# CaNS-World/CaLES

Measured on AMD Instinct MI355X. Metric: time-steps/sec, higher is better.
Workload: dtype f64; 1 GPU; turbulent channel 512x512x512, sgstype=dsmag, PP/PP/NN pressure BCs, bulk forcing in x (BASELINE.json configs[2]); 3 RK substeps/step; decomposition=single GPU

## Files before the change

### cales_amd/csrc/common.hpp

```cpp
#pragma once
#include <hip/hip_runtime.h>
#include <cstdint>
#include <cstdio>
#include <cstdlib>
#include <cstring>
#include <cmath>
#include <string>
#include <vector>
#include "../../include/cales.h"

typedef cales_real real;
#ifdef CALES_SINGLE
typedef float2 real2;
#define CALES_EPS 1.1920929e-07f
#define CALES_BIG 3.4028235e38f
#else
typedef double2 real2;
#define CALES_EPS 2.220446049250313e-16
#define CALES_BIG 1.7976931348623157e308
#endif
constexpr int RSZ = (int)sizeof(real);
constexpr int LINE_REALS = 128 / RSZ;
__host__ __device__ inline real2 make_real2(real x, real y) { real2 r; r.x = x; r.y = y; return r; }

struct Geom {
  int n1, n2, n3;
  int s1;
  long s12;
  int jlo;
  int ng2;

  __host__ __device__ inline size_t ix(int i, int j, int k) const { return (size_t)i + (size_t)s1 * (size_t)j + (size_t)s12 * (size_t)k; }
};

struct DBound { real *x = nullptr, *y = nullptr, *z = nullptr; };
struct RhsBz {
  const real *bc; char ctype, cf; real dlc, dlf, sgn, alpha;
  __host__ __device__ inline real at(int i, int j, int n1) const {
    const real bcv = bc[i + (size_t)(n1 + 2) * j];
    real r = 0.;
    if (cf == 'c') { if (ctype == 'D') r = -2. * bcv / dlc / dlf; else if (ctype == 'N') r = sgn * bcv / dlf; }
    else           { if (ctype == 'D') r = -bcv / dlc / dlf;      else if (ctype == 'N') r = sgn * bcv / dlc; }
    return r * alpha;
  }
};

struct Comm {
  cales_halo_cb halo = nullptr; cales_alltoall_cb a2a = nullptr; cales_allreduce_cb allred = nullptr; void *user = nullptr;
  real *A = nullptr, *B = nullptr; int64_t nbuf = 0;
  bool on = false;
  cales_halo_s_cb halo_s = nullptr; cales_alltoall_part_cb a2a_part = nullptr;
  bool halo_second_stream = false, a2a_second_stream = false, has_lo = false, has_hi = false;
};

struct Spec {
  int blocked, cw, n2l, n3;
  int nyq = 0;
  __host__ __device__ inline size_t at_slab(const Geom &g, int m, int jl, int k) const {
    if (!blocked) return (g.ix(0, jl, k) >> 1) + (size_t)m;
    const int peer = m / cw, mm = m - peer * cw;
    return (size_t)mm + (size_t)cw * ((size_t)(jl - 1) + (size_t)n2l * ((size_t)(k - 1) + (size_t)n3 * peer));
  }
  __host__ __device__ inline size_t at_mode(const Geom &g, int mm, int j, int k) const {
    if (!blocked) return (g.ix(0, j, k) >> 1) + (size_t)mm;
    const int peer = (j - 1) / n2l, jl = (j - 1) - peer * n2l;
    return (size_t)mm + (size_t)cw * ((size_t)jl + (size_t)n2l * ((size_t)(k - 1) + (size_t)n3 * peer));
  }
};

struct Flags {
  bool unfolded_correc = false, unfolded_mom = false, eager_projection = false, lazy_projection = false, helmholtz_z_per_column = false, unfused_imp_rhs = false, unfused_correc = false, unfused_forcing = false, unfused_fillps = false, unfused_mean = false, keep_last_rhs = false, wide_offsets = false, dsmag_reference_sequence = false, dsmag_xghosts = false, smag_reference_sequence = false, gaussel_march = false, fft_generic = false, fft_no_odd_radix = false, keep_null_mode = false, unfused_rk = false, overlap = false, xghosts_in_step = false, unmerged_bc = false, no_nyquist_packing = false, sgs_six_components = false;
  int kchunk = 0; long tile_min_blocks = 2048;
  std::string test_bad_launch;
  void read_env() {
    test_bad_launch = getenv("CALES_TEST_BAD_LAUNCH") ? getenv("CALES_TEST_BAD_LAUNCH") : "";
    unfolded_mom = getenv("CALES_UNFOLDED_MOM") != nullptr;
    lazy_projection = getenv("CALES_LAZY_PROJECTION") != nullptr;
    eager_projection = getenv("CALES_EAGER_PROJECTION") != nullptr;
    unfolded_correc = getenv("CALES_UNFOLDED_CORREC") != nullptr;
    helmholtz_z_per_column = getenv("CALES_HELMHOLTZ_Z_PER_COLUMN") != nullptr;
    unfused_imp_rhs = getenv("CALES_UNFUSED_IMP_RHS") != nullptr;
    unfused_correc = getenv("CALES_UNFUSED_CORREC") != nullptr;
    unfused_forcing = getenv("CALES_UNFUSED_FORCING") != nullptr;
    unfused_fillps = getenv("CALES_UNFUSED_FILLPS") != nullptr;
    unfused_mean = getenv("CALES_UNFUSED_MEAN") != nullptr;
    keep_last_rhs = getenv("CALES_KEEP_LAST_RHS") != nullptr;
    wide_offsets = getenv("CALES_WIDE_OFFSETS") != nullptr;
    dsmag_reference_sequence = getenv("CALES_DSMAG_REFERENCE_SEQUENCE") != nullptr;
    dsmag_xghosts = getenv("CALES_DSMAG_XGHOSTS") != nullptr;
    sgs_six_components = getenv("CALES_SGS_SIX_COMPONENTS") != nullptr;
    smag_reference_sequence = getenv("CALES_SMAG_REFERENCE_SEQUENCE") != nullptr;
    gaussel_march = getenv("CALES_GAUSSEL_MARCH") != nullptr;
    no_nyquist_packing = getenv("CALES_NO_NYQUIST_PACKING") != nullptr;
    fft_generic = getenv("CALES_FFT_GENERIC") != nullptr;
    fft_no_odd_radix = getenv("CALES_FFT_NO_ODD_RADIX") != nullptr;
    xghosts_in_step = getenv("CALES_XGHOSTS_IN_STEP") != nullptr;
    keep_null_mode = getenv("CALES_KEEP_NULL_MODE") != nullptr;
    unfused_rk = getenv("CALES_UNFUSED_RK") != nullptr;
    overlap = getenv("CALES_OVERLAP") != nullptr && atoi(getenv("CALES_OVERLAP")) != 0 && getenv("CALES_NO_OVERLAP") == nullptr;
    unmerged_bc = getenv("CALES_UNMERGED_BC") != nullptr;
    kchunk = getenv("CALES_KCHUNK") ? atoi(getenv("CALES_KCHUNK")) : 0;
    tile_min_blocks = getenv("CALES_TILE_MIN_BLOCKS") ? atol(getenv("CALES_TILE_MIN_BLOCKS")) : 2048;
  }
};

struct StepPlan {
  bool valid = false;
  bool in_visct_zero = false, in_sgs_first = false;
  bool xskip = false;
  bool fold_correc = false;
  bool fold_rows2 = false;
  bool fold_mom = false;
  bool lazy_last = false;
  bool defer_imp_rhs = false;
  bool any_wm = false, skip_first_wm = false;
  bool fuse_cu = false;
  bool defer_force = false;
  bool fuse_fill = false;
  bool visct_ghosts = false;
  bool keep_last_rhs = false;
  int mean_mask = 0, force_mask = 0;
};

struct BandMap { int gx, gy, gz, sub; };
struct TileGeom { dim3 block, grid; int kchunk = 0; BandMap bm{0, 0, 0, 0}; };

enum class SgsForm { none, smag_rows, smag_reference, dsmag_tiles, dsmag_reference };
enum class StrainKernel { corr_rows2, corr, corr5, yw32, yw64, pair, plain32, plain64, f2d32, f2d64 };
enum class LmfKernel { pair, pair5, yw_ucf32, yw_ucf64, yw32, yw64, ucf32, ucf64, plain32, plain64, f2d32, f2d64 };
enum class SmagKernel { yw32, yw64, plain32, plain64 };
enum class SgsAve { planes, volume, xlines };
struct SgsPath {
  SgsForm form = SgsForm::none;
  bool pair = false, lazy = false, ucf = false, small = false, yw = false;
  bool five = false;
  bool filter2d = false;
  SgsAve ave = SgsAve::planes;
  bool wraps_x = true;
  int zlo = 0, zhi = 0, wmlo = 0, wmhi = 0, wylo = 0, wyhi = 0, wmylo = 0, wmyhi = 0; real flo = 0., fhi = 0.;
  int perz = 0, perx = 0, skipz = 0, lmf_ty = 0;
  StrainKernel strain = StrainKernel::plain64; LmfKernel lmf = LmfKernel::plain64; SmagKernel smag = SmagKernel::plain64;
  TileGeom strain_geo, corr_geo, corr_rows2_geo, lmf_geo, smag_geo;
};
struct SgsFold { real dtrk; bool rows2; int fmask; };

struct MomPath {
  bool fused = true;
  int imp = 0;
  bool small = false;
  TileGeom geo;
  bool wm = false, wm_ghosts_in_step = false;
};
struct PendingProjection { real dtrk = 0.; int fmask = 0; bool p_done = false, xskip = false; };

struct BcRule { char t0, t1, cen; real dr0, dr1; const real *bc0, *bc1; };
// ... 329 lines not shown
```

### cales_amd/csrc/k_solver.hip

```cpp
#include "common.hpp"

struct __attribute__((aligned(2 * sizeof(real)))) cpx { real x, y; };
__device__ inline cpx cadd(cpx a, cpx b) { return {a.x + b.x, a.y + b.y}; }
__device__ inline cpx csub(cpx a, cpx b) { return {a.x - b.x, a.y - b.y}; }
__device__ inline cpx cmul(cpx a, cpx b) { return {a.x * b.x - a.y * b.y, a.x * b.y + a.y * b.x}; }
__device__ inline cpx cconj(cpx a) { return {a.x, -a.y}; }
template <int INV> __device__ inline cpx mul_mi(cpx a) { return INV ? cpx{-a.y, a.x} : cpx{a.y, -a.x}; }

template <int R, int INV>
__device__ inline void fft_stage(const cpx *__restrict__ in, cpx *__restrict__ out, int N, int Ns, int t, int T, const cpx *__restrict__ tw) {
  const int M = N / R, tstep = N / (Ns * R);
  for (int j = t; j < M; j += T) {
    const int k = j % Ns;
    cpx v[R];
#pragma unroll
    for (int r = 0; r < R; ++r) v[r] = in[j + r * M];
    if (Ns > 1) {
#pragma unroll
      for (int r = 1; r < R; ++r) { cpx w = tw[k * r * tstep]; if (INV) w.y = -w.y; v[r] = cmul(v[r], w); }
    }
    const int j0 = (j - k) * R + k;
    if (R == 2) {
      out[j0] = cadd(v[0], v[1]); out[j0 + Ns] = csub(v[0], v[1]);
    } else if (R == 4) {
// ... 197 lines not shown
#pragma unroll
    for (int b = 0; b < 4; ++b) { buf[lpad(j0[b])] = v[b][0]; buf[lpad(j0[b] + Ns)] = v[b][1]; }
    __syncthreads();
  }
}

__device__ inline int lmap(int i) { return i; }
template <int INV>
__device__ inline void fft_line8_dif(int N, cpx *buf, int t, const cpx *__restrict__ tw, cpx *v) {
  const int T = N >> 3;
  int R0 = N; while ((R0 & 7) == 0) R0 >>= 3;
  int Nsp;
  if (R0 == 1) {
    fft8_regs<INV>(v);
    if (T == 1) return;
#pragma unroll
    for (int r = 1; r < 8; ++r) v[r] = tw_mul<INV>(v[r], tw[t * r]);
    Nsp = T >> 3;
  } else if (R0 == 4) {
#pragma unroll
    for (int b = 0; b < 2; ++b) {
      const cpx a0 = cadd(v[b], v[b + 4]), a1 = csub(v[b], v[b + 4]), a2 = cadd(v[b + 2], v[b + 6]), a3 = mul_mi<INV>(csub(v[b + 2], v[b + 6]));
      const int j = t + b * T;
      v[b] = cadd(a0, a2); v[b + 2] = tw_mul<INV>(cadd(a1, a3), tw[j]); v[b + 4] = tw_mul<INV>(csub(a0, a2), tw[2 * j]); v[b + 6] = tw_mul<INV>(csub(a1, a3), tw[3 * j]);
    }
    Nsp = T >> 2;
  } else {
#pragma unroll
    for (int b = 0; b < 4; ++b) {
      const cpx x0 = v[b], x1 = v[b + 4];
      v[b] = cadd(x0, x1); v[b + 4] = tw_mul<INV>(csub(x0, x1), tw[t + b * T]);
    }
    Nsp = T >> 1;
  }
  while (true) {
#pragma unroll
    for (int e = 0; e < 8; ++e) buf[lmap(t + e * T)] = v[e];
    __syncthreads();
    const int k = t % Nsp, base = (t - k) * 8 + k, tstep = N / (Nsp * 8);
#pragma unroll
    for (int r = 0; r < 8; ++r) v[r] = buf[lmap(base + r * Nsp)];
    fft8_regs<INV>(v);
    if (Nsp == 1) break;
#pragma unroll
    for (int r = 1; r < 8; ++r) v[r] = tw_mul<INV>(v[r], tw[k * r * tstep]);
    __syncthreads();
    Nsp >>= 3;
  }
}

__device__ inline int dct_src(int e, int n) { return e < n / 2 ? 2 * e : 2 * (n - 1 - e) + 1; }
struct FillArgs { const real *u, *v, *w, *dzfi; real dti, dtidxi, dtidyi; int mean_mask; const real *gvr_f, *gvr_c; real *part; int pstride = 0, pofs = 0; int xwrap = 0; };
template <int INV, int KIND, int FILL = 0, int ODD = 0>
__global__ __launch_bounds__(256, (KIND == 1 && FILL == 1) ? 2 : 1) void k_fft_x8(Geom g, int nh, int iters, const cpx *__restrict__ twg, const cpx *__restrict__ twpg,
                                                 const cpx *__restrict__ twd, real *__restrict__ p, real scale, Spec S, real2 *__restrict__ spec,
                                                 FillArgs F = FillArgs{}, long rbeg = 0, long rend = -1) {
  extern __shared__ __align__(16) unsigned char smem[];
  constexpr int kind = KIND;
  const int T = nh >> 3, R = blockDim.x / T, row = threadIdx.x / T, t = threadIdx.x % T, ld = lpad(nh) + 2;
  cpx *tw = reinterpret_cast<cpx *>(smem), *twp = tw + nh;
  cpx *twl = twp + nh + 1;
  cpx *A = twl + (kind ? nh + 1 : 0) + (size_t)row * ld;
  for (int q = threadIdx.x; q < nh; q += blockDim.x) tw[q] = twg[q];
  for (int q = threadIdx.x; q <= nh; q += blockDim.x) twp[q] = twpg[q];
  if (kind) for (int q = threadIdx.x; q <= nh; q += blockDim.x) twl[q] = twd[q];
  const long nrows = rend < 0 ? (long)g.n2 * g.n3 : rend;
  const int NE = 8;
  cpx nxt[NE + 1];
  real macc[3] = {0., 0., 0.};
  auto rowptr = [&](long r, int &j, int &k) { j = (int)(r % g.n2) + 1; k = (int)(r / g.n2) + 1; };
  auto fetch = [&](long r) {
    if (r >= nrows) return;
    int j, k; rowptr(r, j, k);
    if (!INV && FILL) {
      const size_t c0 = g.ix(0, j, k);
      const real dz = F.dzfi[k];
#pragma unroll
      for (int e = 0; e < NE; ++e) {
        const size_t c = c0 + 1 + 2 * (t + e * T);
        const real2 uu = *reinterpret_cast<const real2 *>(F.u + c); const real um = (F.xwrap && t + e * T == 0) ? F.u[c0 + F.xwrap] : F.u[c - 1];
        const real2 vv = *reinterpret_cast<const real2 *>(F.v + c), vm = *reinterpret_cast<const real2 *>(F.v + c - g.s1);
        const real2 ww = *reinterpret_cast<const real2 *>(F.w + c), wm = *reinterpret_cast<const real2 *>(F.w + c - g.s12);
        nxt[e] = cpx{((ww.x - wm.x) * F.dti * dz + (vv.x - vm.x) * F.dtidyi + (uu.x - um) * F.dtidxi),
                     ((ww.y - wm.y) * F.dti * dz + (vv.y - vm.y) * F.dtidyi + (uu.y - uu.x) * F.dtidxi)};
        if (F.mean_mask & 1) macc[0] += (uu.x + uu.y) * F.gvr_f[k];
        if (F.mean_mask & 2) macc[1] += (vv.x + vv.y) * F.gvr_f[k];
        if (F.mean_mask & 4) macc[2] += (ww.x + ww.y) * F.gvr_c[k];
      }
    } else if (!INV) {
      const real *rowp = p + g.ix(0, j, k);
#pragma unroll
      for (int e = 0; e < NE; ++e) { const int q = t + e * T; nxt[e] = cpx{rowp[1 + 2 * q], rowp[2 + 2 * q]}; }
    } else if (!kind) {
#pragma unroll
      for (int e = 0; e < NE; ++e) { const real2 v = spec[S.at_slab(g, t + e * T, j, k)]; nxt[e] = cpx{v.x, v.y}; }
      if (t == 0) {
        if (S.nyq) { nxt[NE] = cpx{nxt[0].y, 0.}; nxt[0].y = 0.; }
        else { const real2 v = spec[S.at_slab(g, nh, j, k)]; nxt[NE] = cpx{v.x, v.y}; }
      }
    } else {
#pragma unroll
      for (int e = 0; e < NE; ++e) { const real2 v = spec[S.at_slab(g, t + e * T, j, k)]; nxt[e] = cpx{v.x, v.y}; }
    }
  };
  long r = rbeg + ((long)blockIdx.x * iters) * R + row;
  fetch(r);
  for (int it = 0; it < iters; ++it, r += R) {
    const bool live = r < nrows;
    int j = 1, k = 1; if (live) rowptr(r, j, k);
    if (kind && !INV) {
      real *Ad = reinterpret_cast<real *>(A);
#pragma unroll
      for (int e = 0; e < NE; ++e) {
        const int q = t + e * T, r = 2 * nh - 1 - q;
        Ad[2 * lpad(q >> 1) + (q & 1)] = nxt[e].x; Ad[2 * lpad(r >> 1) + (r & 1)] = nxt[e].y;
      }
    } else {
#pragma unroll
      for (int e = 0; e < NE; ++e) A[lpad(t + e * T)] = nxt[e];
    }
    if (INV && !kind && t == 0) A[lpad(nh)] = nxt[NE];
    __syncthreads();
    if (it + 1 < iters) fetch(r + R);
    if (INV && kind) {
      const real *Ad = reinterpret_cast<const real *>(A); const int n = 2 * nh;
      auto coef = [&](int kk) {
        const real yk = Ad[2 * lpad(kk >> 1) + (kk & 1)];
        const int r2 = n - kk; const real ym = kk == 0 ? 0. : Ad[2 * lpad(r2 >> 1) + (r2 & 1)];
        return cmul(cconj(twl[kk]), cpx{yk, -ym});
      };
      cpx xk[NE + 1];
#pragma unroll
      for (int e = 0; e < NE; ++e) xk[e] = coef(t + e * T);
      if (t == 0) xk[NE] = coef(nh);
      __syncthreads();
#pragma unroll
      for (int e = 0; e < NE; ++e) A[lpad(t + e * T)] = xk[e];
      if (t == 0) A[lpad(nh)] = xk[NE];
      __syncthreads();
    }
    real *rowp = p + g.ix(0, j, k);
    if (!INV) {
      fft_line8<0, ODD>(nh, A, t, tw);
      if (live) {
        for (int kk = t; kk <= nh / 2; kk += T) {
          const cpx zk = A[lpad(kk)], zm = cconj(A[lpad((nh - kk) % nh)]);
          const cpx E = {(real)(0.5 * (zk.x + zm.x)), (real)(0.5 * (zk.y + zm.y))};
          const cpx D = csub(zk, zm), O = {(real)(0.5 * D.y), (real)(-0.5 * D.x)};
          const cpx wO = cmul(twp[kk], O);
          const cpx xk = cadd(E, wO), xm = cconj(csub(E, wO));
          if (!kind) {
            if (S.nyq && kk == 0) spec[S.at_slab(g, 0, j, k)] = make_real2(xk.x, xm.x);
            else {
            spec[S.at_slab(g, kk, j, k)] = make_real2(xk.x, xk.y);
            spec[S.at_slab(g, nh - kk, j, k)] = make_real2(xm.x, xm.y);
            }
          } else {
            real *sd = reinterpret_cast<real *>(spec);
            const int n = 2 * nh, k2 = nh - kk;
            const cpx a = cmul(twl[kk], xk), b2 = cmul(twl[k2], xm);
            auto put = [&](int rr, real val) { if (rr < n) sd[2 * S.at_slab(g, rr >> 1, j, k) + (rr & 1)] = val; };
            put(kk, 2. * a.x); if (kk) put(n - kk, -2. * a.y);
            put(k2, 2. * b2.x); if (k2 && k2 != n - k2) put(n - k2, -2. * b2.y);
          }
        }
      }
    } else {
      for (int kk = t; kk <= nh / 2; kk += T) {
        const cpx xa = A[lpad(kk)], xb = A[lpad(nh - kk)];
        const cpx Sa = cadd(xa, cconj(xb)), Da = csub(xa, cconj(xb)), wa = cmul(cconj(twp[kk]), Da);
        const cpx Sb = cadd(xb, cconj(xa)), Db = csub(xb, cconj(xa)), wb = cmul(cconj(twp[nh - kk]), Db);
        const cpx za = cpx{Sa.x - wa.y, Sa.y + wa.x}, zb = cpx{Sb.x - wb.y, Sb.y + wb.x};
        A[lpad(kk)] = za;
        if (kk != 0 && 2 * kk != nh) A[lpad(nh - kk)] = zb;
      }
      __syncthreads();
      fft_line8<1, ODD>(nh, A, t, tw);
      if (live) {
#pragma unroll
        for (int e = 0; e < NE; ++e) {
          const int q = t + e * T;
          if (kind) {
            const real *Ad = reinterpret_cast<const real *>(A); const int r = 2 * nh - 1 - q;
            rowp[1 + 2 * q] = Ad[2 * lpad(q >> 1) + (q & 1)] * scale; rowp[2 + 2 * q] = Ad[2 * lpad(r >> 1) + (r & 1)] * scale;
          } else { const cpx z = A[lpad(q)]; rowp[1 + 2 * q] = z.x * scale; rowp[2 + 2 * q] = z.y * scale; }
        }
      }
    }
    __syncthreads();
  }
  if (FILL && F.mean_mask) {
    real *red = reinterpret_cast<real *>(smem);
#pragma unroll
    for (int q = 0; q < 3; ++q) {
      if (!(F.mean_mask >> q & 1)) continue;
      real v = macc[q];
      if constexpr (ODD) {
        red[threadIdx.x] = v;
        __syncthreads();
        if (threadIdx.x < 64) {
          v = 0.; for (unsigned i = threadIdx.x; i < blockDim.x; i += 64) v += red[i];
          for (int o = 32; o > 0; o >>= 1) v += __shfl_down(v, o, 64);
          if (threadIdx.x == 0) F.part[(size_t)q * (F.pstride ? F.pstride : gridDim.x) + F.pofs + blockIdx.x] = v;
        }
        __syncthreads();
        continue;
      }
      for (int o = 32; o > 0; o >>= 1) v += __shfl_down(v, o, 64);
      if ((threadIdx.x & 63) == 0) red[threadIdx.x >> 6] = v;
      __syncthreads();
      if (threadIdx.x == 0) { real a = 0.; for (unsigned w = 0; w < blockDim.x / 64; ++w) a += red[w]; F.part[(size_t)q * (F.pstride ? F.pstride : gridDim.x) + F.pofs + blockIdx.x] = a; }
      __syncthreads();
    }
  }
}

template <int DIR>
__global__ __launch_bounds__(256) void k_dst1(Geom g, FftPlan P, int ncols, const cpx *__restrict__ tw, real *__restrict__ p, real scale,
                                              Spec S, real2 *__restrict__ pc, int kind = 5, int bwd = 0) {
// ... 499 lines not shown
  real z = 1. / (b[0] + lam + CALES_EPS), d = c[0] * z;
  real v = p[e0] * z;
  p[e0] = v; dscr[s0] = d;
  for (int l = 1; l < nz; ++l) {
    const real bb = b[l] + lam;
    z = 1. / (bb - a[l] * d + CALES_EPS);
    d = c[l] * z;
    v = (p[e0 + l * st] - a[l] * v) * z;
    if (l == nz - 1 && fixnull && lam == 0.) v = 0.;
    p[e0 + l * st] = v; dscr[s0 + l * sst] = d;
  }
  for (int l = nz - 2; l >= 0; --l) {
    v = p[e0 + l * st] - dscr[s0 + l * sst] * v;
    p[e0 + l * st] = v;
  }
}

__device__ inline real rcp_nr(real x) {
  real r = __builtin_amdgcn_rcp(x);
  r = fma(r, fma(-x, r, 1.), r);
  return fma(r, fma(-x, r, 1.), r);
}
__global__ void k_abc_chunked(int nz, int M, const real *__restrict__ a, const real *__restrict__ b, const real *__restrict__ c, real *__restrict__ t, int nch = 64) {
  const int k = blockIdx.x * 256 + threadIdx.x;
  if (k >= nch * M) return;
  const int o = (k % M) * nch + k / M;
  t[o] = (k > 0 && k < nz) ? a[k] : 0.; t[nch * M + o] = k < nz ? b[k] : 1.; t[2 * nch * M + o] = k < nz - 1 ? c[k] : 0.;
}
struct TileMap { int blocked, cw, n2l, mofs, nmode; size_t kstride, segstride; int nyq = 0;
                
                 int nolam, nq, has_lo, has_hi; const real *dud, *force; RhsBz blo, bhi; real hf12; };
constexpr int gt_width(int, int) { return 16; }
#ifndef GT_TL
#define GT_TL 1
#endif
#ifndef GT_PAD
#define GT_PAD 9
#endif
template <int M, int NV, int PER, int DUD = 0>
__global__ __launch_bounds__(64 * gt_width(M, NV) / NV, (PER ? 2 : M <= 8 ? 4 : NV == 1 ? 4 : 2)) void k_gaussel_tile(Geom g, int nz, int ndbl, real lscale, const real *__restrict__ abc,
                                                            const real *__restrict__ lamx, const real *__restrict__ lamy,
                                                            real *__restrict__ p, int fixnull, TileMap T,
                                                            const real *__restrict__ ra = nullptr, const real *__restrict__ rb_ = nullptr, const real *__restrict__ rc = nullptr) {
  extern __shared__ real shz[];
  const int nsys = PER ? nz - 1 : nz;
  constexpr int W = gt_width(M, NV), CP = M + 1, P = 64 * CP + GT_PAD, NT = 64 * W / NV;
  const int t = threadIdx.x;
  const int tile = blockIdx.x;
  const size_t base = (T.blocked ? T.segstride * blockIdx.y : g.ix(0, blockIdx.y + 1, 1)) + (size_t)W * tile;
  const size_t kst = T.blocked ? T.kstride : (size_t)g.s12;
  constexpr bool TL = GT_TL && M == 16;
  real *tabl = shz + W * P;
  if (TL) { for (int q = t; q < 64 * M; q += NT) { tabl[q] = abc[q]; tabl[64 * M + q] = abc[128 * M + q]; } }
  {
    constexpr int W2 = W / 2, KP2 = NT / W2, NQ2 = 64 * M / KP2;
    const int x = 2 * (t % W2), kk = t / W2;
    const bool ok = W * tile + x < ndbl;
    real2 v[NQ2];
#pragma unroll
    for (int q = 0; q < NQ2; ++q) {
      const int k = kk + KP2 * q;
      v[q] = (ok && k < nz) ? *reinterpret_cast<const real2 *>(p + base + x + (size_t)k * kst) : make_real2(0., 0.);
    }
    if (NV == 2 && DUD) {
      const real f = T.force ? T.force[0] : 0.;
      const int bi = ok ? W * tile + x + 1 : 1, bj = (int)blockIdx.y + 1;
      const size_t osafe = base + (ok ? x : 0);
      real2 dd[NQ2], ex[NQ2];
#pragma unroll
      for (int q = 0; q < NQ2; ++q) {
        const int k = kk + KP2 * q;
        dd[q] = *reinterpret_cast<const real2 *>(T.dud + ((ok && k < T.nq) ? base + x + (size_t)k * kst : osafe));
      }
      if (T.nq > nz) {
#pragma unroll
        for (int q = 0; q < NQ2; ++q) {
          const int k = kk + KP2 * q;
          ex[q] = *reinterpret_cast<const real2 *>(p + ((ok && k >= nz && k < T.nq) ? base + x + (size_t)k * kst : osafe));
        }
      }
      real2 lo = make_real2(0., 0.), hi = lo;
      if (T.has_lo) lo = make_real2(T.blo.at(bi, bj, g.n1), T.blo.at(bi + 1, bj, g.n1));
      if (T.has_hi) hi = make_real2(T.bhi.at(bi, bj, g.n1), T.bhi.at(bi + 1, bj, g.n1));
#pragma unroll
      for (int q = 0; q < NQ2; ++q) {
        const int k = kk + KP2 * q;
        const bool in = ok && k < T.nq;
        const real2 own = k < nz ? v[q] : ex[q];
        real2 t = make_real2(own.x - T.hf12 * dd[q].x, own.y - T.hf12 * dd[q].y);
        if (T.force) { t.x = t.x + f; t.y = t.y + f; }
        if (k == 0) { t.x = t.x + lo.x; t.y = t.y + lo.y; }
        if (k == nz - 1) { t.x = t.x + hi.x; t.y = t.y + hi.y; }
        if (in && k < nz) v[q] = t;
        if (in && k >= nz) *reinterpret_cast<real2 *>(p + base + x + (size_t)k * kst) = t;
      }
    }
#pragma unroll
    for (int q = 0; q < NQ2; ++q) { const int k = kk + KP2 * q; shz[x * P + k + k / M] = v[q].x; shz[(x + 1) * P + k + k / M] = v[q].y; }
  }
  __syncthreads();
  const int x = (t >> 6) * NV, ch = t & 63, d = W * tile + x;
  int mode = NV == 1 ? d : d >> 1, j = blockIdx.y + 1;
  bool colok = d < ndbl;
  if (T.blocked) {
    const int f = d >> 1, mm = f % T.cw, jl = f / T.cw;
    j = blockIdx.y * T.n2l + jl + 1;
    mode = NV == 1 ? 2 * (mm + T.mofs) + (d & 1) : mm + T.mofs;
    colok = colok && mm + T.mofs < T.nmode;
  }
  if (T.nyq && mode == 0) colok = false;
  if (colok) {
    const real lam = T.nolam ? 0. : (lamx[mode] + lamy[j - 1]) * lscale;
    const bool nullc = fixnull && lam == 0.;
    real *col = shz + x * P + ch * CP;
    const int k0 = ch * M;
    real cp[M - 1], V[M - 1];
    real cprev = 0., vprev = 0., rprev[NV] = {};
    real pnr[NV] = {}, E[PER ? M - 1 : 1] = {}, eprev = 0.;
    const real e_first = PER ? -ra[0] : 0., e_last = PER ? -rc[nsys - 1] : 0.;
    if (PER) {
#pragma unroll
      for (int q = 0; q < NV; ++q) pnr[q] = shz[(x + q) * P + (nz - 1) + (nz - 1) / M];
    }
#pragma unroll
    for (int r = 0; r < M - 1; ++r) {
      const int k = k0 + r;
      const bool pin = !PER && nullc && k == nz - 1, live = k < nsys && !pin;
      const real A0 = TL ? tabl[r * 64 + ch] : abc[r * 64 + ch], C0 = TL ? tabl[64 * M + r * 64 + ch] : abc[128 * M + r * 64 + ch], B0 = abc[64 * M + r * 64 + ch];
      const real A = pin ? 0. : A0, C = pin ? 0. : C0, B = pin ? 1. : B0 + (k < nsys ? lam : 0.);
      const real z = rcp_nr(B - A * cprev + CALES_EPS);
      cp[r] = C * z; V[r] = (r == 0 ? A : -A * vprev) * z;
#pragma unroll
      for (int q = 0; q < NV; ++q) { const real D0 = col[q * P + r], D = live ? D0 : 0.; rprev[q] = (D - A * rprev[q]) * z; col[q * P + r] = rprev[q]; }
      if (PER) { const real D2 = (k == 0 ? e_first : 0.) + (k == nsys - 1 ? e_last : 0.); eprev = (D2 - A * eprev) * z; E[r] = eprev; }
      cprev = cp[r]; vprev = V[r];
    }
    real Vb = V[M - 2], Wb = cp[M - 2], Rb[NV], Eb = eprev;
#pragma unroll
    for (int q = 0; q < NV; ++q) Rb[q] = rprev[q];
#pragma unroll
    for (int r = M - 3; r >= 0; --r) {
      Vb = V[r] - cp[r] * Vb; Wb = -cp[r] * Wb;
#pragma unroll
      for (int q = 0; q < NV; ++q) Rb[q] = col[q * P + r] - cp[r] * Rb[q];
      if (PER) Eb = E[r] - cp[r] * Eb;
    }
    const bool last = ch == 63;
    real Vn = __shfl_down(Vb, 1, 64), Wn = __shfl_down(Wb, 1, 64);
    if (last) { Vn = 0.; Wn = 0.; }
    real al, be, ga, de[NV], de2 = 0.;
    {
      const int k = k0 + M - 1, r = M - 1;
      const bool pin = !PER && nullc && k == nz - 1, live = k < nsys && !pin;
      const real A0 = TL ? tabl[r * 64 + ch] : abc[r * 64 + ch], C0 = TL ? tabl[64 * M + r * 64 + ch] : abc[128 * M + r * 64 + ch], B0 = abc[64 * M + r * 64 + ch];
      const real A = pin ? 0. : A0, C = pin ? 0. : C0, B = pin ? 1. : B0 + (k < nsys ? lam : 0.);
      al = -A * V[M - 2]; be = B - A * cp[M - 2] - C * Vn; ga = -C * Wn;
      if (PER) {
        real En = __shfl_down(Eb, 1, 64);
        if (last) En = 0.;
        const real D2 = (k == 0 ? e_first : 0.) + (k == nsys - 1 ? e_last : 0.);
        de2 = D2 - A * eprev - C * En;
      }
#pragma unroll
      for (int q = 0; q < NV; ++q) {
        real Rn = __shfl_down(Rb[q], 1, 64);
        if (last) Rn = 0.;
        const real D0 = col[q * P + M - 1], D = live ? D0 : 0.;
        de[q] = D - A * rprev[q] - C * Rn;
      }
    }
#pragma unroll
    for (int h = 1; h < 64; h <<= 1) {
      const bool lo = ch >= h, hi = ch + h < 64;
      const real rb = rcp_nr(be);
      const real rbm = __shfl_up(rb, h, 64), rbp = __shfl_down(rb, h, 64);
      const real k1 = lo ? al * rbm : 0., k2 = hi ? ga * rbp : 0.;
      const real alm = __shfl_up(al, h, 64), gam = __shfl_up(ga, h, 64), alp = __shfl_down(al, h, 64), gap = __shfl_down(ga, h, 64);
      be = be - gam * k1 - alp * k2;
#pragma unroll
      for (int q = 0; q < NV; ++q) de[q] = de[q] - __shfl_up(de[q], h, 64) * k1 - __shfl_down(de[q], h, 64) * k2;
      if (PER) de2 = de2 - __shfl_up(de2, h, 64) * k1 - __shfl_down(de2, h, 64) * k2;
      al = -alm * k1; ga = -gap * k2;
    }
    const real rb = rcp_nr(be);
    const int cL = PER ? (nsys - 1) / M : 0, rL = PER ? (nsys - 1) % M : 0;
    real Es = 0., e1 = 0., eL = 0.;
    if (PER) {
      Es = de2 * rb;
      real sp2 = __shfl_up(Es, 1, 64);
      if (ch == 0) sp2 = 0.;
      real xv2 = eprev - V[M - 2] * sp2 - cp[M - 2] * Es;
      E[M - 2] = xv2;
#pragma unroll
      for (int r = M - 3; r >= 0; --r) { xv2 = E[r] - V[r] * sp2 - cp[r] * xv2; E[r] = xv2; }
      real mine = Es;
#pragma unroll
      for (int r = 0; r < M - 1; ++r) if (r == rL) mine = E[r];
      e1 = __shfl(E[0], 0, 64); eL = __shfl(mine, cL, 64);
    }
#pragma unroll
    for (int q = 0; q < NV; ++q) {
      const real s = de[q] * rb;
      real sp = __shfl_up(s, 1, 64);
      if (ch == 0) sp = 0.;
      real xv = rprev[q] - V[M - 2] * sp - cp[M - 2] * s;
      real mine = (rL == M - 2) ? xv : s;
      col[q * P + M - 2] = xv;
// ... 686 lines not shown
    Y.k = YKernel::fft_y4; if (!make_plan(n2g / 2, Y.plan)) { c->err = std::string(who) + ": ng(2)/2 must factor into primes <= 127"; return 1; }
    Y.lds = stockham_block(4, (size_t)2 * 2 * (n2g / 2 + 1) * sizeof(cpx), &Y.cols);
    if (Y.lds > 64 * 1024) { c->err = std::string(who) + ": y line too long for the LDS-resident DCT-IV"; return 1; }
    if (!s.tw4y && upload_dct4_weights(c, n2g, &s.tw4y)) return 1;
    if (!s.twy4 && upload_twiddles(c, n2g / 2, n2g / 2, &s.twy4)) return 1;
    Y.tw = (const cpx *)s.twy4; Y.twd = (const cpx *)s.tw4y; Y.fn.y4[0] = Y.fn.y4[1] = P.ykind == 3 ? k_fft_y4<0> : k_fft_y4<1>; return 0; }
  Y.k = YKernel::fft_y;
  if (!make_plan(n2g, Y.plan)) { c->err = "solver: ng(1)/2 and ng(2) must factor into primes <= 127"; return 1; }
  Y.lds = stockham_block(8, (size_t)2 * (n2g + 1) * sizeof(cpx), &Y.cols);
  if (Y.lds > 64 * 1024) { c->err = "solver: line too long for the LDS-resident transform"; return 1; }
  Y.fn.y[0] = k_fft_y<0>; Y.fn.y[1] = k_fft_y<1>; return 0;
}
static int choose_kernels(cales_ctx *c, Solver &s, SolvePath &P, const char *who) {
  if (x_pass(c, s, P) || y_pass(c, s, P, who)) return 1;
  const bool hasd = CBP(c, 0, 3) == 'D' || CBP(c, 1, 3) == 'D';
  P.fixnull = (P.poisson && !hasd && !c->fl.keep_null_mode) ? 1 : 0; P.refnull = P.poisson && !hasd && c->fl.keep_null_mode; P.null_switch = c->fl.keep_null_mode;
  if (P.xkind && !P.ykind) P.zk = ZKernel::herm;
  else if ((P.periodic_z || P.fixnull || !P.poisson || hasd) && tile_takes(c, P.nz, P.periodic_z)) P.zk = ZKernel::tile;
  else if (P.xkind) P.zk = P.periodic_z ? ZKernel::periodic_real : ZKernel::ri;
  else P.zk = P.periodic_z ? ZKernel::periodic_cpx : ZKernel::ri;
  return 0;
}
static void tile_setup(cales_ctx *c, SolvePath &P, real *tab) {
  if (P.zk != ZKernel::tile) return;
  ZTile &Z = P.zt; Z.M = tile_m(P.nz); Z.NV = P.xkind ? 1 : 2; Z.PER = P.periodic_z ? 1 : 0; Z.tab = tab;
  Z.ndbl = c->P > 1 ? 2 * P.cw * c->n[1] : P.xkind ? 2 * (c->C.ng[0] / 2) : 2 * (P.nyq ? c->n[0] / 2 : c->n[0] / 2 + 1); Z.nrow = c->P > 1 ? c->P : c->C.ng[1];
  Z.persistent = !Z.PER && Z.NV == 1 && P.nz == 1024 && Z.ndbl % 16 == 0;
  tile_attr(c, Z);
}
static int solve_sched(cales_ctx *c, const SolvePath &P, SolveSched &D) {
  D = SolveSched();
  const int *n = c->n, mh = n[0] / 2 + 1, n2g = c->C.ng[1], nh = c->C.ng[0] / 2, cw = P.cw;
  const bool dist = c->P > 1, use8x = P.xp.k == XKernel::fft_x8, use8y = radix8_y(P.yp.k), use16y = P.yp.k == YKernel::fft_y16;
  const int Rx8 = use8x ? P.xp.rows : 1, CB8 = use8y ? P.yp.cols : 1;
  if (dist) { D.slab_spec = reinterpret_cast<real2 *>(c->comm.A); D.mode_spec = reinterpret_cast<real2 *>(c->comm.B); }
  D.nmodes = P.nyq ? n[0] / 2 : mh; D.ncol = dist ? cw : D.nmodes; D.mofs = dist ? c->rank * cw : 0;
  D.ncol_y = (!dist && P.xkind == 1 && use8y) ? nh : D.ncol;
  D.S.blocked = dist ? 1 : 0; D.S.cw = cw; D.S.n2l = n[1]; D.S.n3 = n[2]; D.S.nyq = P.nyq ? 1 : 0;
  D.T.blocked = dist ? 1 : 0; D.T.cw = cw; D.T.n2l = n[1]; D.T.mofs = D.mofs; D.T.nmode = P.xkind ? nh : D.nmodes; D.T.nyq = P.nyq ? 1 : 0; D.T.kstride = (size_t)2 * cw * n[1]; D.T.segstride = D.T.kstride * n[2];
  D.gz = P.zk == ZKernel::herm ? dim3((unsigned)(((long)4 * D.ncol * (n2g / 2 + 1) + 255) / 256)) : P.zk == ZKernel::ri ? dim3((unsigned)(((long)2 * D.ncol * n2g + 255) / 256))
       : dim3(((P.zk == ZKernel::periodic_real ? 2 * nh : D.ncol) + 63) / 64, (n2g + 3) / 4);
  if (c->comm.a2a_second_stream && use8x && use8y) { if (n[2] % 4 == 0 && n[2] >= 32) D.nch = 4; else if (n[2] % 2 == 0 && n[2] >= 8) D.nch = 2; }
  const bool pipe = D.nch > 1;
  D.kpc = n[2] / D.nch; D.rows = (long)n[1] * D.kpc;
  D.a2a_stride = (int64_t)n[2] * n[1] * cw * 2; D.a2a_chunk = (int64_t)D.kpc * n[1] * cw * 2;
  if (dist && c->P * D.a2a_stride > c->stage.a2a) {
    c->err = "solver: an all-to-all of " + std::to_string(c->P) + " blocks of " + std::to_string(D.a2a_stride) + " reals does not fit the " + std::to_string(c->stage.a2a) + " the staging buffers were sized for";
    return 1;
  }
  const long xgroups = (D.rows + Rx8 - 1) / Rx8;
  int xiters = 1; while (xiters < 8 && xgroups / (xiters * 2) >= 2048 / D.nch) xiters *= 2;
  if (!pipe && xgroups <= 8192) xiters = 1;
  D.xit_f = xiters; D.xit_b = (!pipe && P.xkind == 0 && nh <= 256) ? 1 : xiters;
  D.xblk_f = (unsigned)((xgroups + D.xit_f - 1) / D.xit_f); D.xblk_b = (unsigned)((xgroups + D.xit_b - 1) / D.xit_b); D.npart = (int)(D.xblk_f * D.nch);
  { const long cg = (D.ncol + CB8 - 1) / CB8, from = pipe ? 2048 / D.nch : 8192;
    while (D.ykc < 8 && cg * (D.kpc / (D.ykc * 2)) >= from && D.kpc % (D.ykc * 2) == 0) D.ykc *= 2; }
  if (use16y) {
    const long slots = (long)(c->ncu > 0 ? c->ncu : 256) * (n2g >= 1024 ? 1 : n2g >= 512 ? 2 : 4), tiles = (D.ncol_y + 7) / 8;
    double best = 1e300;
    for (int kc = 1; kc <= 32 && kc <= D.kpc; ++kc) {
      const long nb = tiles * ((D.kpc + kc - 1) / kc);
      const double cost = (double)((nb + slots - 1) / slots) * (kc + 1.5);
      if (cost < best) { best = cost; D.ykc = kc; }
    }
  }
  return 0;
}
int solver_comm_changed(cales_ctx *c) {
  Solver *s = c->solver;
  if (!s) return 0;
  if (solve_sched(c, s->pres, s->sched_pres)) return 1;
  for (int iv = 0; iv < 3; ++iv) if (s->vel_state[iv] == 1 && solve_sched(c, s->vel[iv], s->sched_vel[iv])) return 1;
  ctx_free(c, s->d_mpart); s->d_mpart = nullptr;
  const bool forced = c->C.is_forced[0] || c->C.is_forced[1] || c->C.is_forced[2];
  return (forced && s->pres.xp.k == XKernel::fft_x8) ? ctx_alloc(c, &s->d_mpart, 3 * (size_t)s->sched_pres.npart, false) : 0;
}

int solver_setup(cales_ctx *c) {
  Solver &s = *(c->solver = new Solver());
  SolvePath &P = s.pres;
  const int *n = c->n; const int n1 = c->C.ng[0], n2g = c->C.ng[1], n3 = n[2];
  P.xkind = line_kind(&c->C.cbcpre[0], false); P.ykind = line_kind(&c->C.cbcpre[2], false);
  if (P.xkind < 0 || P.ykind < 0) { c->err = "solver: unknown pressure BC pair in x or y"; return 1; }
  if (P.ykind >= 3 && (n2g % 2)) { c->err = "solver: ND/DN in y need an even ng(2)"; return 1; }
  if (P.xkind && c->C.cbcpre[4] == 'P' && (!P.ykind || c->P > 1)) { c->err = "solver: a non-periodic x with periodic z needs a non-periodic y and one rank"; return 1; }
  if (upload_twiddles(c, n1 / 2, n1 / 2, &s.twx)) return 1;
  if (upload_twiddles(c, n1, n1 / 2 + 1, &s.twx_post)) return 1;
  if (upload_twiddles(c, n2g, n2g, &s.twy)) return 1;
  if (upload_twiddles(c, 4 * n1, n1 / 2 + 1, &s.twy_post)) return 1;
  if (upload_twiddles(c, 4 * n2g, n2g, &s.twyd)) return 1;
  const int mh = n1 / 2 + 1;
  c->cw = (mh + c->P - 1) / c->P;
  if (c->P > 1) { const int cw8 = (c->cw + 7) / 8 * 8; if (100 * (cw8 - c->cw) <= 6 * c->cw && (size_t)cw8 * n2g * n3 <= c->ntot) c->cw = cw8; }
  if (c->P > 1 && (size_t)c->cw * n2g * n3 > c->ntot) { c->err = "solver: scratch too small for the mode-block layout"; return 1; }
  P.nz = n3; P.periodic_z = CBP(c, 0, 3) == 'P' && CBP(c, 1, 3) == 'P'; P.poisson = true;
  if (choose_kernels(c, s, P, "solver")) return 1;
  { const bool hasd = CBP(c, 0, 3) == 'D' || CBP(c, 1, 3) == 'D';
    P.nyq = P.xkind == 0 && P.ykind <= 1 && P.xp.k == XKernel::fft_x8 && radix8_y(P.yp.k) && !P.periodic_z && (hasd || !c->fl.keep_null_mode) && tile_takes(c, n3, false) && !c->fl.no_nyquist_packing;
    if (P.nyq && P.zk != ZKernel::tile) { c->err = "solver: the packed mode column needs the z solve in the LDS tile"; return 1; }
    P.cw = P.nyq ? (n1 / 2 + c->P - 1) / c->P : c->cw; }
  { double nx, ny;
    if (line_spectrum(c, 0, &c->C.cbcpre[0], false, P.xkind, &P.lamx, &nx) || line_spectrum(c, 1, &c->C.cbcpre[2], false, P.ykind, &P.lamy, &ny)) return 1; P.normfft = 1. / (nx * ny); }
  std::vector<real> abc(3 * (size_t)n3);
  hs_tridmatrix(&c->C.cbcpre[4], n3, c->dzci.data(), c->dzfi.data(), 'c', abc.data(), abc.data() + n3, abc.data() + 2 * n3);
  if (ctx_upload(c, &s.d_a, abc)) return 1;
  s.d_b = s.d_a + n3; s.d_c = s.d_a + 2 * n3;
// ... 294 lines not shown
```

Measured before the change: 27.43 time-steps/s.

## Split fused divergence prefetch in x-FFT to overlap loads with FFT compute

The fused fill-and-forward x-FFT kernel now fetches the next row's divergence inputs in two halves. The second half's loads are issued before the current row's FFT post-processing and reduced after it, to hide global memory latency. Launch bounds now request 2 blocks/SM for all FILL variants. The tridiagonal solver caches its coefficients in registers for small M. An env knob to override x-FFT rows per block is also added. The extra register arrays risk spills or lower occupancy.

```diff
diff --git a/cales_amd/csrc/common.hpp b/cales_amd/csrc/common.hpp
--- a/cales_amd/csrc/common.hpp
+++ b/cales_amd/csrc/common.hpp
@@ -71,6 +71,7 @@
 struct Flags {
   bool unfolded_correc = false, unfolded_mom = false, eager_projection = false, lazy_projection = false, helmholtz_z_per_column = false, unfused_imp_rhs = false, unfused_correc = false, unfused_forcing = false, unfused_fillps = false, unfused_mean = false, keep_last_rhs = false, wide_offsets = false, dsmag_reference_sequence = false, dsmag_xghosts = false, smag_reference_sequence = false, gaussel_march = false, fft_generic = false, fft_no_odd_radix = false, keep_null_mode = false, unfused_rk = false, overlap = false, xghosts_in_step = false, unmerged_bc = false, no_nyquist_packing = false, sgs_six_components = false;
   int kchunk = 0; long tile_min_blocks = 2048;
+  int x_row_groups[2] = {0, 0};
   std::string test_bad_launch;
   void read_env() {
     test_bad_launch = getenv("CALES_TEST_BAD_LAUNCH") ? getenv("CALES_TEST_BAD_LAUNCH") : "";
@@ -101,6 +102,8 @@
     unmerged_bc = getenv("CALES_UNMERGED_BC") != nullptr;
     kchunk = getenv("CALES_KCHUNK") ? atoi(getenv("CALES_KCHUNK")) : 0;
     tile_min_blocks = getenv("CALES_TILE_MIN_BLOCKS") ? atol(getenv("CALES_TILE_MIN_BLOCKS")) : 2048;
+    x_row_groups[0] = x_row_groups[1] = 0;
+    if (const char *e = getenv("CALES_X_ROW_GROUPS")) { if (sscanf(e, "%d,%d", &x_row_groups[0], &x_row_groups[1]) < 2) x_row_groups[1] = x_row_groups[0]; }
   }
 };
 
diff --git a/cales_amd/csrc/k_solver.hip b/cales_amd/csrc/k_solver.hip
--- a/cales_amd/csrc/k_solver.hip
+++ b/cales_amd/csrc/k_solver.hip
@@ -273,7 +273,7 @@
 __device__ inline int dct_src(int e, int n) { return e < n / 2 ? 2 * e : 2 * (n - 1 - e) + 1; }
 struct FillArgs { const real *u, *v, *w, *dzfi; real dti, dtidxi, dtidyi; int mean_mask; const real *gvr_f, *gvr_c; real *part; int pstride = 0, pofs = 0; int xwrap = 0; };
 template <int INV, int KIND, int FILL = 0, int ODD = 0>
-__global__ __launch_bounds__(256, (KIND == 1 && FILL == 1) ? 2 : 1) void k_fft_x8(Geom g, int nh, int iters, const cpx *__restrict__ twg, const cpx *__restrict__ twpg,
+__global__ __launch_bounds__(256, FILL == 1 ? 2 : 1) void k_fft_x8(Geom g, int nh, int iters, const cpx *__restrict__ twg, const cpx *__restrict__ twpg,
                                                  const cpx *__restrict__ twd, real *__restrict__ p, real scale, Spec S, real2 *__restrict__ spec,
                                                  FillArgs F = FillArgs{}, long rbeg = 0, long rend = -1) {
   extern __shared__ __align__(16) unsigned char smem[];
@@ -290,45 +290,58 @@
   cpx nxt[NE + 1];
   real macc[3] = {0., 0., 0.};
   auto rowptr = [&](long r, int &j, int &k) { j = (int)(r % g.n2) + 1; k = (int)(r / g.n2) + 1; };
+  constexpr int E0 = 6, ER = NE - E0 > E0 ? NE - E0 : E0;
+  real2 ruu[ER], rvv[ER], rvm[ER], rww[ER], rwm[ER]; real rum[ER], rdz = 0., rgf = 0., rgc = 0.; bool rin = false;
+  auto fill_row = [&](long r) {
+    rin = r < nrows; int j, k; rowptr(rin ? r : nrows - 1, j, k);
+    rdz = F.dzfi[k]; rgf = F.gvr_f[k]; rgc = F.gvr_c[k];
+  };
+  auto fill_issue = [&](long r, int e0, int e1) {
+    int j, k; rowptr(r < nrows ? r : nrows - 1, j, k);
+    const size_t c0 = g.ix(0, j, k);
+#pragma unroll
+    for (int i = 0; i < ER; ++i) {
+      if (e0 + i >= e1) break;
+      const int q = t + (e0 + i) * T;
+      const size_t c = c0 + 1 + 2 * q;
+      ruu[i] = *reinterpret_cast<const real2 *>(F.u + c); rum[i] = F.u[(F.xwrap && q == 0) ? c0 + F.xwrap : c - 1];
+      rvv[i] = *reinterpret_cast<const real2 *>(F.v + c); rvm[i] = *reinterpret_cast<const real2 *>(F.v + c - g.s1);
+      rww[i] = *reinterpret_cast<const real2 *>(F.w + c); rwm[i] = *reinterpret_cast<const real2 *>(F.w + c - g.s12);
+    }
+  };
+  auto fill_reduce = [&](int e0, int e1) {
+#pragma unroll
+    for (int i = 0; i < ER; ++i) {
+      if (e0 + i >= e1) break;
+      const real2 uu = ruu[i], vv = rvv[i], vm = rvm[i], ww = rww[i], wm = rwm[i]; const real um = rum[i], dz = rdz;
+      nxt[e0 + i] = cpx{((ww.x - wm.x) * F.dti * dz + (vv.x - vm.x) * F.dtidyi + (uu.x - um) * F.dtidxi),
+                        ((ww.y - wm.y) * F.dti * dz + (vv.y - vm.y) * F.dtidyi + (uu.y - uu.x) * F.dtidxi)};
+      if (rin && (F.mean_mask & 1)) macc[0] += (uu.x + uu.y) * rgf;
+      if (rin && (F.mean_mask & 2)) macc[1] += (vv.x + vv.y) * rgf;
+      if (rin && (F.mean_mask & 4)) macc[2] += (ww.x + ww.y) * rgc;
+    }
+  };
   auto fetch = [&](long r) {
-    if (r >= nrows) return;
-    int j, k; rowptr(r, j, k);
-    if (!INV && FILL) {
-      const size_t c0 = g.ix(0, j, k);
-      const real dz = F.dzfi[k];
-#pragma unroll
-      for (int e = 0; e < NE; ++e) {
-        const size_t c = c0 + 1 + 2 * (t + e * T);
-        const real2 uu = *reinterpret_cast<const real2 *>(F.u + c); const real um = (F.xwrap && t + e * T == 0) ? F.u[c0 + F.xwrap] : F.u[c - 1];
-        const real2 vv = *reinterpret_cast<const real2 *>(F.v + c), vm = *reinterpret_cast<const real2 *>(F.v + c - g.s1);
-        const real2 ww = *reinterpret_cast<const real2 *>(F.w + c), wm = *reinterpret_cast<const real2 *>(F.w + c - g.s12);
-        nxt[e] = cpx{((ww.x - wm.x) * F.dti * dz + (vv.x - vm.x) * F.dtidyi + (uu.x - um) * F.dtidxi),
-                     ((ww.y - wm.y) * F.dti * dz + (vv.y - vm.y) * F.dtidyi + (uu.y - uu.x) * F.dtidxi)};
-        if (F.mean_mask & 1) macc[0] += (uu.x + uu.y) * F.gvr_f[k];
-        if (F.mean_mask & 2) macc[1] += (vv.x + vv.y) * F.gvr_f[k];
-        if (F.mean_mask & 4) macc[2] += (ww.x + ww.y) * F.gvr_c[k];
-      }
-    } else if (!INV) {
+    int j, k; rowptr(r < nrows ? r : nrows - 1, j, k);
+    if (!INV) {
       const real *rowp = p + g.ix(0, j, k);
 #pragma unroll
       for (int e = 0; e < NE; ++e) { const int q = t + e * T; nxt[e] = cpx{rowp[1 + 2 * q], rowp[2 + 2 * q]}; }
-    } else if (!kind) {
+    } else {
 #pragma unroll
       for (int e = 0; e < NE; ++e) { const real2 v = spec[S.at_slab(g, t + e * T, j, k)]; nxt[e] = cpx{v.x, v.y}; }
-      if (t == 0) {
-        if (S.nyq) { nxt[NE] = cpx{nxt[0].y, 0.}; nxt[0].y = 0.; }
-        else { const real2 v = spec[S.at_slab(g, nh, j, k)]; nxt[NE] = cpx{v.x, v.y}; }
-      }
-    } else {
-#pragma unroll
-      for (int e = 0; e < NE; ++e) { const real2 v = spec[S.at_slab(g, t + e * T, j, k)]; nxt[e] = cpx{v.x, v.y}; }
+      if (!kind && !S.nyq) { const real2 v = spec[S.at_slab(g, nh, j, k)]; nxt[NE] = cpx{v.x, v.y}; }
     }
   };
   long r = rbeg + ((long)blockIdx.x * iters) * R + row;
-  fetch(r);
+  if (!INV && FILL) {
+    fill_row(r);
+    fill_issue(r, 0, E0); fill_reduce(0, E0); fill_issue(r, E0, NE); fill_reduce(E0, NE);
+  } else fetch(r);
   for (int it = 0; it < iters; ++it, r += R) {
-    const bool live = r < nrows;
+    const bool live = r < nrows, more = it + 1 < iters;
     int j = 1, k = 1; if (live) rowptr(r, j, k);
+    if (INV && !kind && S.nyq && t == 0) { nxt[NE] = cpx{nxt[0].y, 0.}; nxt[0].y = 0.; }
     if (kind && !INV) {
       real *Ad = reinterpret_cast<real *>(A);
 #pragma unroll
@@ -342,7 +355,9 @@
     }
     if (INV && !kind && t == 0) A[lpad(nh)] = nxt[NE];
     __syncthreads();
-    if (it + 1 < iters) fetch(r + R);
+    if (more) {
+      if (!INV && FILL) { fill_row(r + R); fill_issue(r + R, 0, E0); fill_reduce(0, E0); } else fetch(r + R);
+    }
     if (INV && kind) {
       const real *Ad = reinterpret_cast<const real *>(A); const int n = 2 * nh;
       auto coef = [&](int kk) {
@@ -363,6 +378,7 @@
     real *rowp = p + g.ix(0, j, k);
     if (!INV) {
       fft_line8<0, ODD>(nh, A, t, tw);
+      if (FILL && more) fill_issue(r + R, E0, NE);
       if (live) {
         for (int kk = t; kk <= nh / 2; kk += T) {
           const cpx zk = A[lpad(kk)], zm = cconj(A[lpad((nh - kk) % nh)]);
@@ -386,6 +402,7 @@
           }
         }
       }
+      if (FILL && more) fill_reduce(E0, NE);
     } else {
       for (int kk = t; kk <= nh / 2; kk += T) {
         const cpx xa = A[lpad(kk)], xb = A[lpad(nh - kk)];
@@ -991,6 +1008,8 @@
   constexpr bool TL = GT_TL && M == 16;
   real *tabl = shz + W * P;
   if (TL) { for (int q = t; q < 64 * M; q += NT) { tabl[q] = abc[q]; tabl[64 * M + q] = abc[128 * M + q]; } }
+  constexpr bool TR = M <= 8 && !PER && !DUD;
+  real tA[TR ? M : 1], tB[TR ? M : 1], tC[TR ? M : 1];
   {
     constexpr int W2 = W / 2, KP2 = NT / W2, NQ2 = 64 * M / KP2;
     const int x = 2 * (t % W2), kk = t / W2;
@@ -1000,6 +1019,10 @@
     for (int q = 0; q < NQ2; ++q) {
       const int k = kk + KP2 * q;
       v[q] = (ok && k < nz) ? *reinterpret_cast<const real2 *>(p + base + x + (size_t)k * kst) : make_real2(0., 0.);
+    }
+    if (TR) {
+#pragma unroll
+      for (int r = 0; r < M; ++r) { tA[r] = abc[r * 64 + (t & 63)]; tB[r] = abc[64 * M + r * 64 + (t & 63)]; tC[r] = abc[128 * M + r * 64 + (t & 63)]; }
     }
     if (NV == 2 && DUD) {
       const real f = T.force ? T.force[0] : 0.;
@@ -1065,7 +1088,7 @@
     for (int r = 0; r < M - 1; ++r) {
       const int k = k0 + r;
       const bool pin = !PER && nullc && k == nz - 1, live = k < nsys && !pin;
-      const real A0 = TL ? tabl[r * 64 + ch] : abc[r * 64 + ch], C0 = TL ? tabl[64 * M + r * 64 + ch] : abc[128 * M + r * 64 + ch], B0 = abc[64 * M + r * 64 + ch];
+      const real A0 = TR ? tA[r] : TL ? tabl[r * 64 + ch] : abc[r * 64 + ch], C0 = TR ? tC[r] : TL ? tabl[64 * M + r * 64 + ch] : abc[128 * M + r * 64 + ch], B0 = TR ? tB[r] : abc[64 * M + r * 64 + ch];
       const real A = pin ? 0. : A0, C = pin ? 0. : C0, B = pin ? 1. : B0 + (k < nsys ? lam : 0.);
       const real z = rcp_nr(B - A * cprev + CALES_EPS);
       cp[r] = C * z; V[r] = (r == 0 ? A : -A * vprev) * z;
@@ -1091,7 +1114,7 @@
     {
       const int k = k0 + M - 1, r = M - 1;
       const bool pin = !PER && nullc && k == nz - 1, live = k < nsys && !pin;
-      const real A0 = TL ? tabl[r * 64 + ch] : abc[r * 64 + ch], C0 = TL ? tabl[64 * M + r * 64 + ch] : abc[128 * M + r * 64 + ch], B0 = abc[64 * M + r * 64 + ch];
+      const real A0 = TR ? tA[r] : TL ? tabl[r * 64 + ch] : abc[r * 64 + ch], C0 = TR ? tC[r] : TL ? tabl[64 * M + r * 64 + ch] : abc[128 * M + r * 64 + ch], B0 = TR ? tB[r] : abc[64 * M + r * 64 + ch];
       const real A = pin ? 0. : A0, C = pin ? 0. : C0, B = pin ? 1. : B0 + (k < nsys ? lam : 0.);
       al = -A * V[M - 2]; be = B - A * cp[M - 2] - C * Vn; ga = -C * Wn;
       if (PER) {
@@ -1884,6 +1907,8 @@
   int xiters = 1; while (xiters < 8 && xgroups / (xiters * 2) >= 2048 / D.nch) xiters *= 2;
   if (!pipe && xgroups <= 8192) xiters = 1;
   D.xit_f = xiters; D.xit_b = (!pipe && P.xkind == 0 && nh <= 256) ? 1 : xiters;
+  if (c->fl.x_row_groups[0] >= 1 && c->fl.x_row_groups[0] <= 64) D.xit_f = c->fl.x_row_groups[0];
+  if (c->fl.x_row_groups[1] >= 1 && c->fl.x_row_groups[1] <= 64) D.xit_b = c->fl.x_row_groups[1];
   D.xblk_f = (unsigned)((xgroups + D.xit_f - 1) / D.xit_f); D.xblk_b = (unsigned)((xgroups + D.xit_b - 1) / D.xit_b); D.npart = (int)(D.xblk_f * D.nch);
   { const long cg = (D.ncol + CB8 - 1) / CB8, from = pipe ? 2048 / D.nch : 8192;
     while (D.ykc < 8 && cg * (D.kpc / (D.ykc * 2)) >= from && D.kpc % (D.ykc * 2) == 0) D.ykc *= 2; }
```

Result: no change. 27.52 time-steps/s (median of 2 runs) (+0.3%).
